# NVIDIA/retinanet-examples

Measured on AMD Instinct MI355X. Metric: images/sec end-to-end (incl. decode+NMS), RN50FPN 800px bs=8, higher is better.
Workload: dtype bf16; 1 GPU; ResNet50FPN bf16 inference, bs=8 per GPU at 800x1280, HIP decode x5 + NMS; global_batch=8, parallelism=replicas x1 (no data-path collective), entry=Model.forward (eval), postproc=fused

## Files before the change

include/odtk_hip.h:

```cpp
#ifndef ODTK_HIP_H
#define ODTK_HIP_H

#include <stddef.h>
#include <stdint.h>

#ifdef __cplusplus
extern "C" {
#endif

#define ODTK_OK                0
#define ODTK_ERR_INVALID      -1
#define ODTK_ERR_WORKSPACE    -2
#define ODTK_ERR_HIP          -3
#define ODTK_ERR_UNSUPPORTED  -4

#define ODTK_MAX_LEVELS    6
#define ODTK_MAX_ANCHORS   32
#define ODTK_ATSS_MAX_TOPK 16
#define ODTK_MAX_TOP_N     16384
#define ODTK_MAX_NMS_COUNT 7680
#define ODTK_MAX_NMS_COUNT_SCRATCH (1 << 22)
#define ODTK_MAX_NMS_DETECTIONS 2048

#define ODTK_F32   0
// ... 125 lines not shown
int odtk_preprocess_images(int batch_size, const odtk_image_t *images, const void *src, size_t src_bytes, const int32_t *tables,
                           size_t tables_len, const void *norm_table, void *out, int height, int width, int dtype, void *stream);

#define ODTK_AUGMENT_BRIGHTNESS 1u
#define ODTK_AUGMENT_CONTRAST   2u
#define ODTK_AUGMENT_HUE        4u
#define ODTK_AUGMENT_SATURATION 8u
typedef struct odtk_augment {
  int32_t canvas_width, canvas_height;
  int32_t map[6];
  uint32_t flags;
  float brightness, contrast, saturation;
  uint8_t hue;
  uint8_t pad_[3];
} odtk_augment_t;
int odtk_augment_images(int batch_size, const odtk_image_t *images, const odtk_augment_t *augments, const void *src, size_t src_bytes,
                        const int32_t *tables, size_t tables_len, const void *norm_table, void *out, int height, int width, int dtype,
                        void *workspace, size_t workspace_bytes, void *stream);
typedef struct odtk_rotation {
  double matrix[6];
  int32_t enabled;
  int32_t flip;
} odtk_rotation_t;
int odtk_augment_images_ex(int batch_size, const odtk_image_t *images, const odtk_augment_t *augments, const odtk_rotation_t *rotations,
                           const void *src, size_t src_bytes, const int32_t *tables, size_t tables_len, const void *norm_table, void *out,
                           int height, int width, int dtype, void *workspace, size_t workspace_bytes, void *stream);
int odtk_gemm_init(const char *hipblaslt_path);
size_t odtk_gemm_plan_export(char *text, size_t capacity);
int odtk_gemm_plan_import(const char *text);
int odtk_gemm_plan_pin_misses(void);
int odtk_gemm_bias_act(void *y, const void *x, const void *w, const float *bias, const void *residual,
                       size_t m, int n, int k, int dtype, int relu,
                       void *workspace, size_t workspace_size, void *stream);

int odtk_snap_to_anchors(int batch_size, const float *targets, int n_max, const float *anchors,
                         int num_anchors, int num_classes, int height, int width, int stride,
                         float iou_background, float iou_foreground,
                         float *cls_target, float *box_target, float *depth, void *stream);

typedef struct odtk_snap_level {
  const float *anchors;
  float *cls_target;
  float *box_target;
  float *depth;
  int32_t height, width, stride, pad_;
} odtk_snap_level_t;
int odtk_snap_to_anchors_levels(int batch_size, const float *targets, int n_max, int n_levels,
                                const odtk_snap_level_t *levels, int num_anchors, int num_classes,
                                float iou_background, float iou_foreground, void *stream);

int odtk_atss_assign_levels(int batch_size, const float *targets, int n_max, int n_levels,
                            const odtk_snap_level_t *levels, int num_anchors, int num_classes, int topk,
                            void *workspace, size_t workspace_size, void *stream);

typedef struct odtk_snap_rot_level {
  const float *anchors_axis;
  const float *anchors_quads;
  float *cls_target;
  float *box_target;
  float *depth;
  int32_t height, width, stride, pad_;
} odtk_snap_rot_level_t;
int odtk_snap_to_anchors_rotated_levels(int batch_size, const float *gt_axis, const float *gt_quads, const float *gt_class,
                                        int n_max, int n_levels, const odtk_snap_rot_level_t *levels, int num_anchors,
                                        int num_classes, float iou_background, float iou_foreground, void *stream);

// ... 15 lines not shown
  void *dcls, *dbox;
  int32_t height, width;
  int32_t channels_last;
  int32_t pad_;
} odtk_loss_level_t;

int odtk_retina_loss_levels_forward(int n_levels, const odtk_loss_level_t *levels, int batch_size, int num_anchors,
                                    int num_classes, int box_params, int dtype, float alpha, float gamma, float beta,
                                    double *sums, void *stream);
int odtk_retina_loss_levels_forward_ws(int n_levels, const odtk_loss_level_t *levels, int batch_size, int num_anchors,
                                       int num_classes, int box_params, int dtype, float alpha, float gamma, float beta,
                                       double *sums, void *workspace, size_t workspace_size, void *stream);
int odtk_retina_loss_levels_backward(int n_levels, const odtk_loss_level_t *levels, int batch_size, int num_anchors,
                                     int num_classes, int box_params, int dtype, float alpha, float gamma, float beta,
                                     const float *grad_cls_sums, const float *grad_box_sums, void *stream);

#define ODTK_KERNEL_PREFILTER 0
#define ODTK_KERNEL_SELECT    1
#define ODTK_KERNEL_NMS       2
#define ODTK_KERNEL_IOU       3
#define ODTK_KERNEL_EPILOGUE  4
#define ODTK_KERNEL_TARGETS   5
#define ODTK_KERNEL_GEMM      6
#define ODTK_KERNEL_LOSS      7
#define ODTK_KERNEL_SELHIST   8
#define ODTK_KERNEL_SELFILTER 9
#define ODTK_KERNEL_NMS_ORDER 10
#define ODTK_KERNEL_NMS_MATRIX 11
#define ODTK_KERNEL_POOL      12
#define ODTK_KERNEL_UPSAMPLE  13
#define ODTK_KERNEL_STEM_PACK 14
#define ODTK_KERNEL_LOSS_REDUCE 15
#define ODTK_KERNEL_ATSS_STATS 16
#define ODTK_KERNEL_COUNT     17
int odtk_profile_enable(int on);
int odtk_debug_set_trace(void *device_buffer);
int odtk_debug_loss_tuning(int which, int fp32_heads, int threads, int blocks_per_cu, int unroll, int box_blocks);
int odtk_debug_loss_layout(int which, int fp32_heads, int per_wave, int window, int box_rows);
int odtk_debug_loss_tuning_get(int which, int fp32_heads, int out[7]);
#define ODTK_LOSS_FORM_DEFAULT 1
int odtk_debug_loss_form(int form);
int odtk_debug_loss_form_get(void);
int odtk_profile_collect(double total_ms[ODTK_KERNEL_COUNT], int launches[ODTK_KERNEL_COUNT]);

#ifdef __cplusplus
}
#endif
#endif
```

retinanet-examples_amd/csrc/engine.hip:

```cpp
#include <cstring>

#include "runtime.hpp"
#include "epilogue.hpp"
#include "gemm_lt.hpp"

namespace {

template <typename T, bool kRes, bool kRelu>
int bias_act_launch(void *y, const float *bias, const void *res, uint64_t n, uint32_t channels, hipStream_t stream) {
  constexpr int per = T::kPerLoad;
  uint64_t done = 0;
  if (channels % per == 0 && n / per >= 256) {
    const uint32_t vpr = channels / per;
    const uint64_t n_vec = n / per;
    uint32_t g = vpr, m = 256;
    while (m) { const uint32_t r_ = g % m; g = m; m = r_; }
    const uint32_t unit = vpr / g;
    uint64_t blocks = (n_vec + 256ull * 4 - 1) / (256ull * 4);
    if (blocks > 256 * 16) blocks = 256 * 16;
    blocks = (blocks + unit - 1) / unit * unit;
    timed_launch(ODTK_KERNEL_EPILOGUE, odtk::bias_act_kernel<T, kRes, kRelu>, dim3(static_cast<unsigned>(blocks)), dim3(256), 0,
                 stream, y, bias, res, n_vec, vpr);
    done = n_vec * per;
  }
  if (done < n) {
    uint64_t blocks = (n - done + 255) / 256;
    if (blocks > 4096) blocks = 4096;
    hipLaunchKernelGGL((odtk::bias_act_scalar_kernel<T, kRes, kRelu>), dim3(static_cast<unsigned>(blocks)), dim3(256),
                       0, stream, y, bias, res, done, n, channels);
  }
  ODTK_HIP_TRY(hipGetLastError());
  return ODTK_OK;
}

template <typename T>
int bias_act_typed(void *y, const float *bias, const void *res, uint64_t n, uint32_t c, bool relu, hipStream_t s) {
  if (res) return relu ? bias_act_launch<T, true, true>(y, bias, res, n, c, s) : bias_act_launch<T, true, false>(y, bias, res, n, c, s);
  return relu ? bias_act_launch<T, false, true>(y, bias, res, n, c, s) : bias_act_launch<T, false, false>(y, bias, res, n, c, s);
}

int bias_act_dispatch(void *y, const float *bias, const void *res, uint64_t n, uint32_t c, int dtype, bool relu,
                      hipStream_t s) {
  return dispatch_dtype(dtype, [&](auto t) { return bias_act_typed<decltype(t)>(y, bias, res, n, c, relu, s); });
}

template <typename TIn>
int stem_pack_launch(const void *x, void *out, int batch, int height, int width, int channels_last, int out_dtype, hipStream_t stream) {
  const unsigned long long total = 1ull * batch * (height / 2) * (width / 2);
  unsigned long long blocks = (total + 255) / 256;
  if (blocks > 256 * 32) blocks = 256 * 32;
  const odtk::FastDiv by_wo = odtk::fastdiv_make(static_cast<uint32_t>(width / 2));
  const odtk::FastDiv by_howo = odtk::fastdiv_make(static_cast<uint32_t>(height / 2) * static_cast<uint32_t>(width / 2));
  if (out_dtype == ODTK_BF16)
    timed_launch(ODTK_KERNEL_STEM_PACK, odtk::stem_pack_kernel<TIn, odtk::BF16>, dim3(static_cast<unsigned>(blocks)), dim3(256), 0, stream, x, out,
                 static_cast<uint32_t>(batch), static_cast<uint32_t>(height), static_cast<uint32_t>(width), static_cast<uint32_t>(channels_last), by_wo, by_howo);
  else
    timed_launch(ODTK_KERNEL_STEM_PACK, odtk::stem_pack_kernel<TIn, odtk::F16>, dim3(static_cast<unsigned>(blocks)), dim3(256), 0, stream, x, out,
                 static_cast<uint32_t>(batch), static_cast<uint32_t>(height), static_cast<uint32_t>(width), static_cast<uint32_t>(channels_last), by_wo, by_howo);
  ODTK_HIP_TRY(hipGetLastError());
  return ODTK_OK;
}

}

extern "C" {

int odtk_bias_act(void *y, const float *bias, const void *residual, size_t n_pixels, int channels, int dtype,
                  int relu, void *stream) {
  if (!y || !bias || channels <= 0) return ODTK_ERR_INVALID;
  if (dtype != ODTK_F32 && dtype != ODTK_BF16 && dtype != ODTK_F16) return ODTK_ERR_UNSUPPORTED;
  if ((reinterpret_cast<uintptr_t>(y) & 15u) || (reinterpret_cast<uintptr_t>(residual) & 15u)) return ODTK_ERR_INVALID;
  const uint64_t n = static_cast<uint64_t>(n_pixels) * channels;
  if (n == 0) return ODTK_OK;
  return bias_act_dispatch(y, bias, residual, n, static_cast<uint32_t>(channels), dtype, relu != 0,
                           static_cast<hipStream_t>(stream));
}

int odtk_bias_act_maxpool(const void *y, const float *bias, void *out, int batch_size, int height, int width,
                          int channels, int dtype, int relu, void *stream) {
  if (!y || !bias || !out || batch_size <= 0 || height <= 0 || width <= 0 || channels <= 0) return ODTK_ERR_INVALID;
  if (dtype != ODTK_BF16 && dtype != ODTK_F16) return ODTK_ERR_UNSUPPORTED;
  if (channels % 8 != 0) return ODTK_ERR_UNSUPPORTED;
  if ((reinterpret_cast<uintptr_t>(y) | reinterpret_cast<uintptr_t>(out)) & 15u) return ODTK_ERR_INVALID;
  if (1ull * height * width * channels >= (1ull << 32)) return ODTK_ERR_UNSUPPORTED;
  const uint32_t ho = (static_cast<uint32_t>(height) + 1) / 2, wo = (static_cast<uint32_t>(width) + 1) / 2;
  const uint64_t work = static_cast<uint64_t>(batch_size) * ho * wo * (channels / 8);
  uint64_t blocks = (work + 255) / 256;
  if (blocks > 256 * 32) blocks = 256 * 32;
  hipStream_t s = static_cast<hipStream_t>(stream);
  const uint16_t *in = static_cast<const uint16_t *>(y);
  uint16_t *o = static_cast<uint16_t *>(out);
  odtk::PoolDivisors dv;
  dv.groups = odtk::fastdiv_make(static_cast<uint32_t>(channels / 8));
  dv.wo = odtk::fastdiv_make(wo);
  dv.ho = odtk::fastdiv_make(ho);
  const bool small = work < (1ull << 32);
#define ODTK_POOL_(T, R, S)                                                                                             \
  timed_launch(ODTK_KERNEL_POOL, odtk::bias_act_maxpool_kernel<T, R, S>, dim3(static_cast<unsigned>(blocks)), dim3(256), 0, s, in, \
// ... 103 lines not shown
```

retinanet-examples_amd/odtk/_C.py:

```python
import ctypes
import threading
import os

import torch

_LIB_PATH = os.environ.get('ODTK_HIP_LIBRARY') or os.path.join(os.path.dirname(os.path.abspath(__file__)), 'libodtk_hip.so')

OK, ERR_INVALID, ERR_WORKSPACE, ERR_HIP, ERR_UNSUPPORTED = 0, -1, -2, -3, -4
F32, BF16, F16 = 0, 1, 2
FLAG_ROTATED, FLAG_LOGITS, FLAG_ROTATED_NMS_FIXED_ANGLE = 1, 2, 4
MAX_LEVELS, MAX_ANCHORS, MAX_TOP_N, MAX_NMS_COUNT, MAX_NMS_COUNT_SCRATCH = 6, 32, 16384, 7680, 1 << 22
MAX_CONCAT_PARTS = 8
MAX_TILES = 64
SOFT_NMS_LINEAR, SOFT_NMS_GAUSSIAN = 1, 2
ATSS_MAX_TOPK = 16

_vp = ctypes.c_void_p
_vpp = ctypes.POINTER(ctypes.c_void_p)
_fp = ctypes.POINTER(ctypes.c_float)
_sz = ctypes.c_size_t


class LossLevel(ctypes.Structure):
    _fields_ = [('cls', ctypes.c_void_p), ('box', ctypes.c_void_p), ('depth', ctypes.c_void_p), ('box_target', ctypes.c_void_p),
# ... 92 lines not shown
    'odtk_snap_to_anchors_rotated_levels': (ctypes.c_int, [ctypes.c_int, _vp, _vp, _vp, ctypes.c_int, ctypes.c_int,
                                                           ctypes.POINTER(SnapRotLevel), ctypes.c_int, ctypes.c_int, ctypes.c_float,
                                                           ctypes.c_float, _vp]),
    'odtk_prefilter_thresholds': (ctypes.c_int, [_vp, ctypes.c_int, ctypes.c_int, ctypes.c_float, _vp, _vp]),
    'odtk_upsample_nearest2x': (ctypes.c_int, [ctypes.c_void_p, ctypes.c_void_p, ctypes.c_int, ctypes.c_int, ctypes.c_int, ctypes.c_int,
                                               ctypes.c_int, ctypes.c_void_p]),
    'odtk_canvas_clear': (ctypes.c_int, [ctypes.c_void_p] + [ctypes.c_int] * 5 + [ctypes.POINTER(ctypes.c_int), ctypes.c_int, ctypes.c_void_p]),
    'odtk_canvas_pack': (ctypes.c_int, [ctypes.c_void_p] + [ctypes.c_int] * 5 + [ctypes.POINTER(ctypes.c_int), _vpp, ctypes.c_int,
                                        ctypes.c_void_p]),
    'odtk_stem_pack': (ctypes.c_int, [ctypes.c_void_p, ctypes.c_void_p, ctypes.c_int, ctypes.c_int, ctypes.c_int, ctypes.c_int,
                                      ctypes.c_int, ctypes.c_int, ctypes.c_void_p]),
    'odtk_preprocess_images': (ctypes.c_int, [ctypes.c_int, ctypes.POINTER(Image), _vp, _sz, _vp, _sz, _vp, _vp, ctypes.c_int, ctypes.c_int,
                                              ctypes.c_int, _vp]),
    'odtk_augment_images': (ctypes.c_int, [ctypes.c_int, ctypes.POINTER(Image), ctypes.POINTER(Augment), _vp, _sz, _vp, _sz, _vp, _vp,
                                           ctypes.c_int, ctypes.c_int, ctypes.c_int, _vp, _sz, _vp]),
    'odtk_augment_images_ex': (ctypes.c_int, [ctypes.c_int, ctypes.POINTER(Image), ctypes.POINTER(Augment), ctypes.POINTER(Rotation), _vp, _sz,
                                              _vp, _sz, _vp, _vp, ctypes.c_int, ctypes.c_int, ctypes.c_int, _vp, _sz, _vp]),
    'odtk_nms_sorted_runs': (ctypes.c_int, [ctypes.c_int, _vpp, _vpp, ctypes.c_int, _sz, ctypes.c_int, _vp, ctypes.c_int, ctypes.c_float,
                                            ctypes.c_uint32, _vp, _sz, _vp]),
    'odtk_soft_nms': (ctypes.c_int, [ctypes.c_int, _vpp, _vpp, ctypes.c_int, _sz, ctypes.c_int, ctypes.c_float, ctypes.c_int,
                                     ctypes.c_float, ctypes.c_float, ctypes.c_uint32, _vp, _sz, _vp]),
    'odtk_box_vote': (ctypes.c_int, [ctypes.c_int, _vpp, _vp, _vp, _sz, ctypes.c_int, ctypes.c_float, ctypes.c_uint32, _vp]),
    'odtk_concat_candidates': (ctypes.c_int, [ctypes.c_int, ctypes.c_int, ctypes.POINTER(Candidates), _vpp, ctypes.c_uint32, _vp]),
    'odtk_tile_images': (ctypes.c_int, [_vp, _vp] + [ctypes.c_int] * 7 + [ctypes.POINTER(Tile), ctypes.c_int, ctypes.c_int, _vp]),
    'odtk_merge_tile_candidates': (ctypes.c_int, [ctypes.c_int, ctypes.POINTER(Tile), _vpp, _vpp, _sz] + [ctypes.c_int] * 6 +
                                   [ctypes.c_float, ctypes.c_uint32, _vp]),
    'odtk_gemm_init': (ctypes.c_int, [ctypes.c_char_p]),
    'odtk_gemm_plan_export': (ctypes.c_size_t, [ctypes.c_char_p, ctypes.c_size_t]),
    'odtk_gemm_plan_import': (ctypes.c_int, [ctypes.c_char_p]),
    'odtk_gemm_plan_pin_misses': (ctypes.c_int, []),
    'odtk_gemm_bias_act': (ctypes.c_int, [ctypes.c_void_p, ctypes.c_void_p, ctypes.c_void_p, ctypes.c_void_p, ctypes.c_void_p,
                                          ctypes.c_size_t, ctypes.c_int, ctypes.c_int, ctypes.c_int, ctypes.c_int,
                                          ctypes.c_void_p, ctypes.c_size_t, ctypes.c_void_p]),
    'odtk_profile_collect': (ctypes.c_int, [ctypes.POINTER(ctypes.c_double), ctypes.POINTER(ctypes.c_int)]),
}

KERNEL_NAMES = ('prefilter_scan_kernel', 'select_decode_kernel', 'nms_kernel', 'iou_pairs_kernel', 'bias_act_kernel',
                'snap_to_anchors_kernel', 'gemm_bias_act', 'retina_loss_kernel', 'select_hist_kernel', 'select_filter_kernel',
                'nms_first_round_kernel', 'rotated_sup_matrix_kernel', 'bias_act_maxpool_kernel', 'upsample_nearest2x_kernel',
                'stem_pack_kernel', 'loss_reduce_kernel', 'atss_stats_kernel')
traffic_count = False
traffic_bytes = {}


def _count(name, nbytes):
    if traffic_count:
        traffic_bytes[name] = traffic_bytes.get(name, 0) + int(nbytes)


_lib = None


def library():
    global _lib
    if _lib is None:
        if not os.path.isfile(_LIB_PATH):
            raise ImportError('odtk._C: %s is missing -- build the HIP library first '
                              '(python __graft_entry__.py, or make -C retinanet-examples_amd/csrc). '
                              'There is no CPU fallback.' % _LIB_PATH)
        lib = ctypes.CDLL(_LIB_PATH)
        for name, (res, args) in _SIGNATURES.items():
            fn = getattr(lib, name)
            fn.restype = res
            fn.argtypes = args
        for which, mirror in ((0, Level), (1, SnapLevel), (2, SnapRotLevel), (3, LossLevel), (5, Image), (6, Augment), (7, Rotation),
                              (9, Candidates), (11, Tile)):
            if lib.odtk_abi_struct_size(which) != ctypes.sizeof(mirror):
                raise ImportError('odtk._C: %s was built from another revision of include/odtk_hip.h (sizeof struct %d: library %d, '
                                  'binding %d) -- rebuild it (make -C retinanet-examples_amd/csrc)'
                                  % (_LIB_PATH, which, lib.odtk_abi_struct_size(which), ctypes.sizeof(mirror)))
        _lib = lib
        for part in filter(None, os.environ.get('ODTK_LOSS_TUNING', '').split(';')):
            side, _, vals = part.partition(':')
# ... 716 lines not shown
def gemm_available():
    if not _GEMM_READY:
        shipped = os.path.join(os.path.dirname(torch.__file__), 'lib', 'libhipblaslt.so')
        path = shipped if os.path.exists(shipped) else None
        rc = library().odtk_gemm_init(path.encode() if path else None)
        _GEMM_READY.append(rc == OK)
    return _GEMM_READY[0]


def gemm_bias_act(x, weight, bias, residual=None, relu=True):
    if not x.is_cuda or x.dim() != 4 or x.dtype not in _DTYPES:
        raise RuntimeError('gemm_bias_act: x must be a 4-d CUDA tensor of float32/bfloat16/float16')
    b, k, h, w = x.shape
    n = weight.shape[0]
    if weight.numel() != n * k or weight.dtype != x.dtype or not weight.is_contiguous() and not weight.is_contiguous(
            memory_format=torch.channels_last):
        raise RuntimeError('gemm_bias_act: weight must be a dense [Cout, Cin(, 1, 1)] tensor of x.dtype')
    if not _channels_last(x, True):
        raise RuntimeError('gemm_bias_act: x must be channels_last')
    if not _bias_vector(bias, n):
        raise RuntimeError('gemm_bias_act: bias must be a float32 CUDA vector of length Cout')
    y = torch.empty((b, n, h, w), dtype=x.dtype, device=x.device, memory_format=torch.channels_last)
    if residual is not None and (residual.shape != y.shape or residual.dtype != y.dtype or not _channels_last(residual, True)):
        raise RuntimeError('gemm_bias_act: residual must match the output (shape, dtype, channels_last)')
    with torch.cuda.device(x.device):
        ws, stream = _gemm_setup(x.device)
        _check(library().odtk_gemm_bias_act(y.data_ptr(), x.data_ptr(), weight.data_ptr(), bias.data_ptr(),
                                            residual.data_ptr() if residual is not None else None,
                                            b * h * w, n, k, _DTYPES[x.dtype], 1 if relu else 0,
                                            ws.data_ptr(), ws.numel(), stream), 'gemm_bias_act')
    return y


_CONV_LIB_PATH = os.path.join(os.path.dirname(os.path.abspath(__file__)), 'libodtk_conv.so')
_conv_lib = []


def conv_library():
    if not _conv_lib:
        lib = None
        if os.path.isfile(_CONV_LIB_PATH) and not os.environ.get('ODTK_NO_CONV_LIBRARY'):
            lib = ctypes.CDLL(_CONV_LIB_PATH)
            lib.odtk_conv_bias_act.restype = ctypes.c_int
            lib.odtk_conv_bias_act.argtypes = [ctypes.c_void_p] * 4 + [ctypes.c_int] * 13 + [ctypes.c_void_p]
            lib.odtk_conv_bias_act_pads.restype = ctypes.c_int
            lib.odtk_conv_bias_act_pads.argtypes = [ctypes.c_void_p] * 4 + [ctypes.c_int] * 15 + [ctypes.c_void_p]
            lib.odtk_conv_bias_act_strided.restype = ctypes.c_int
            lib.odtk_conv_bias_act_strided.argtypes = ([ctypes.c_void_p] * 4 + [ctypes.c_int] * 13 + [ctypes.c_longlong] * 6 +
                                                       [ctypes.c_int] * 2 + [ctypes.c_void_p])
            lib.odtk_conv_last_plan.restype = ctypes.c_char_p
            lib.odtk_conv_last_plan.argtypes = []
            lib.odtk_conv_instance_count.restype = ctypes.c_int
            lib.odtk_conv_instance_count.argtypes = [ctypes.c_int]
            lib.odtk_conv_plan_export.restype = ctypes.c_size_t
            lib.odtk_conv_plan_export.argtypes = [ctypes.c_char_p, ctypes.c_size_t]
            lib.odtk_conv_plan_import.restype = ctypes.c_int
            lib.odtk_conv_plan_import.argtypes = [ctypes.c_char_p]
        _conv_lib.append(lib)
    return _conv_lib[0]


def conv_available():
    return conv_library() is not None


def conv_bias_act(x, weight, bias, stride=(1, 1), padding=(1, 1), relu=True, out=None):
# ... 143 lines not shown
```

retinanet-examples_amd/odtk/fused.py:

```python
import hashlib
import json
import os
import threading

import torch
import torch.nn as nn
import torch.nn.functional as F

from . import _C
from . import box as box_ops
from .backbones.resnet import BasicBlock, Bottleneck


_PLAN_LOCK = threading.Lock()
_TLS = threading.local()


def _planning():
    return getattr(_TLS, 'planning', False)


def _key_str(key):
    kind, shape = ('only', key[1:]) if key and key[0] == 'only' else ('act', key)
    return kind + ':' + 'x'.join(str(int(v)) for v in shape)
# ... 183 lines not shown
    def _routed(self, key, kind, x, two, one):
        route = self.route.get(key)
        if route is None and _Conv.route_mode != 'auto':
            route = self.route[key] = (_Conv.route_mode == 'library', None, None)
        if route is None and _planning() and not torch.cuda.is_current_stream_capturing():
            route = self.route[key] = self._measure(x, two, one)
            self.learned[kind] = route[0]
        if route is None:
            return self.learned.get(kind, False)
        return route[0]

    def conv_then_pool(self, x):
        if not x.is_cuda:
            return F.max_pool2d(self._torch(x), 3, 2, 1)
        y = F.conv2d(x, self.weight, None, self.stride, self.padding, groups=self.groups)
        if y.dtype in (torch.bfloat16, torch.float16) and y.shape[1] % 8 == 0:
            return _C.bias_act_maxpool(y.contiguous(memory_format=torch.channels_last), self.bias, self.relu)
        return F.max_pool2d(_C.bias_act_(y.contiguous(memory_format=torch.channels_last), self.bias, None, self.relu), 3, 2, 1)


class _Block(nn.Module):
    def __init__(self, block, dtype):
        super().__init__()
        if isinstance(block, Bottleneck):
            self.convs = nn.ModuleList([_Conv(block.conv1, block.bn1, True, dtype), _Conv(block.conv2, block.bn2, True, dtype)])
            self.last = _Conv(block.conv3, block.bn3, True, dtype)
        elif isinstance(block, BasicBlock):
            self.convs = nn.ModuleList([_Conv(block.conv1, block.bn1, True, dtype)])
            self.last = _Conv(block.conv2, block.bn2, True, dtype)
        else:
            raise TypeError('unsupported block %r' % type(block))
        self.down = None if block.downsample is None else _Conv(block.downsample[0], block.downsample[1], False, dtype)

    def forward(self, x):
        skip = x if self.down is None else self.down(x)
        y = x
        for c in self.convs:
            y = c(y)
        return self.last(y, skip)


class FusedRetinaNet(nn.Module):
    @staticmethod
    def supports(model):
        if len(model.backbones) != 1:
            return False
        fpn = next(iter(model.backbones.values()))
        net = getattr(fpn, 'features', None)
        if net is None or not all(hasattr(net, n) for n in ('conv1', 'bn1', 'layer1', 'layer2', 'layer3', 'layer4')):
            return False
        if list(getattr(net, 'outputs', [])) != [3, 4, 5]:
            return False
        return all(isinstance(b, (Bottleneck, BasicBlock)) for layer in (net.layer1, net.layer2, net.layer3, net.layer4)
                   for b in layer)

    def __init__(self, model, dtype=torch.bfloat16):
        super().__init__()
        if not self.supports(model):
            raise ValueError('FusedRetinaNet supports a single ResNet-FPN backbone')
        fpn = next(iter(model.backbones.values()))
        net = fpn.features
        self.dtype = dtype
        self.model = [model]
        self.stem = _Conv(net.conv1, net.bn1, True, dtype)
        self.stem_s2d = None
        c1 = net.conv1
        if (tuple(c1.kernel_size), tuple(c1.stride), tuple(c1.padding), c1.in_channels, c1.groups) == ((7, 7), (2, 2), (3, 3), 3, 1) \
                and dtype in (torch.bfloat16, torch.float16):
            w = self.stem.weight.float()
            w4 = stem_space_to_depth_weights(w)
            self.register_buffer('stem_w4', w4.to(dtype).contiguous(memory_format=torch.channels_last))
            self.register_buffer('stem_zero_bias', torch.zeros(w.shape[0], dtype=dtype, device=w.device))
            self.stem_s2d = {}
        self.stem_learned = False
        self.layers = nn.ModuleList([nn.ModuleList([_Block(b, dtype) for b in layer])
                                     for layer in (net.layer1, net.layer2, net.layer3, net.layer4)])
        self.outputs = list(net.outputs)
        self.lateral = nn.ModuleList([_Conv(fpn.lateral3, None, False, dtype), _Conv(fpn.lateral4, None, False, dtype),
                                      _Conv(fpn.lateral5, None, False, dtype)])
        self.smooth = nn.ModuleList([_Conv(fpn.smooth3, None, False, dtype), _Conv(fpn.smooth4, None, False, dtype),
                                     _Conv(fpn.smooth5, None, False, dtype)])
        self.pyramid6 = _Conv(fpn.pyramid6, None, False, dtype)
        self.pyramid7 = _Conv(fpn.pyramid7, None, False, dtype)

        def head(seq):
            convs = [m for m in seq if isinstance(m, nn.Conv2d)]
            return nn.ModuleList([_Conv(c, None, i + 1 < len(convs), dtype) for i, c in enumerate(convs)])

        self.cls_head = head(model.cls_head)
        self.box_head = head(model.box_head)
        self.level_streams = True
        self.pyramid_canvas = os.environ.get('ODTK_PYRAMID_CANVAS', '1') != '0'
        self._streams = None
        self.tower_plan = 0
        self._planned = set()
        self._loaded_geometries = set()
        self._plan_file_seen = False
        self.libraries_taken = None
        self.max_plans = 4
        self._graphs = {}
        self._thresholds = {}
        self.max_graphs = 8

    def _stem_direct(self, x):
        x = x.to(self.dtype).contiguous(memory_format=torch.channels_last)
        return self.stem.conv_then_pool(x)

    def _stem_packed(self, x):
        xs = _C.stem_pack(x, self.dtype)
        y = _C.conv_bias_act(xs, self.stem_w4, self.stem_zero_bias, 1, ((2, 1), (2, 1)), False)
        return _C.bias_act_maxpool(y, self.stem.bias, self.stem.relu)

    def _stem(self, x):
        if (self.stem_s2d is not None and _Conv.use_conv_library and x.is_cuda and x.dim() == 4 and x.shape[1] == 3
                and x.shape[2] % 2 == 0 and x.shape[3] % 2 == 0 and x.dtype in _C._DTYPES and _C.conv_available()
                and (x.is_contiguous() or x.is_contiguous(memory_format=torch.channels_last))):
            key = (tuple(x.shape), x.dtype, x.is_contiguous())
            route = self.stem_s2d.get(key)
            if route is None and _Conv.route_mode != 'auto':
                route = self.stem_s2d[key] = (_Conv.route_mode == 'library', None, None)
            if route is None and _planning() and not torch.cuda.is_current_stream_capturing():
                route = self.stem_s2d[key] = self.stem._measure(x, self._stem_direct, self._stem_packed)
                self.stem_learned = route[0]
            if route[0] if route is not None else self.stem_learned:
                try:
                    return self._stem_packed(x)
                except RuntimeError:
                    self.stem_s2d[key] = (False, float('inf'), 0.0)
        return self._stem_direct(x)

    def features(self, x):
        x = self._stem(x)
        feats = []
        for level, layer in enumerate(self.layers, start=2):
            for block in layer:
                x = block(x)
            if level in self.outputs:
                feats.append(x)
        c3, c4, c5 = feats
        p5 = self.lateral[2](c5)
        p4 = self.lateral[1](c4, self._upsample(p5))
        p3 = self.lateral[0](c3, self._upsample(p4))
        p6 = self.pyramid6(c5)
        p7 = self.pyramid7(F.relu(p6))
        return [self.smooth[0](p3), self.smooth[1](p4), self.smooth[2](p5), p6, p7]

    @staticmethod
    def _upsample(t):
        if (t.is_cuda and t.dtype in _C._DTYPES and t.is_contiguous(memory_format=torch.channels_last)
                and (t.shape[1] * t.element_size()) % 16 == 0):
            return _C.upsample2x(t)
        return F.interpolate(t, scale_factor=2).contiguous(memory_format=torch.channels_last)

    @staticmethod
    def _run(seq, t):
        for c in seq:
            t = c(t)
        return t

    def _canvas_gutter(self, feats):
        if not self.pyramid_canvas or len(feats) < 3 or not (feats[0].is_cuda or self.pyramid_canvas == 'always'):
            return None
        gutter = 0
        for c in list(self.cls_head[:-1]) + list(self.box_head[:-1]):
            kh, kw = c.weight.shape[2:]
            if (tuple(c.stride) != (1, 1) or c.groups != 1 or kh % 2 == 0 or kw % 2 == 0 or tuple(c.padding) != (kh // 2, kw // 2)
                    or c.weight.shape[0] != c.weight.shape[1]):
                return None
            gutter = max(gutter, kh // 2, kw // 2)
# ... 67 lines not shown
        ready = torch.cuda.Event()
        ready.record(main)
        done = []
        for stream, group in zip(self._streams, groups):
            stream.wait_event(ready)
            with torch.cuda.stream(stream):
                for i in group:
                    for pair in unit(i):
                        for t in pair:
                            t.record_stream(main)
                e = torch.cuda.Event()
                e.record(stream)
                done.append(e)
        for i in mine:
            unit(i)
        for e in done:
            main.wait_event(e)
        return [o[0] for o in out], [o[1] for o in out]

    def heads(self, x):
        with torch.autocast(x.device.type, enabled=False):
            return self._towers(self.features(x), True)

    def heads_without_last_bias(self, x):
        with torch.autocast(x.device.type, enabled=False):
            cls, box = self._towers(self.features(x), False)
        return cls, box, self.cls_head[-1].bias, self.box_head[-1].bias

    @torch.no_grad()
    def replay(self, x):
        m = self.model[0]
        bias = self.cls_head[-1].bias
        key = (tuple(x.shape), x.dtype, x.device, x.is_contiguous(memory_format=torch.channels_last),
               m.threshold, m.top_n, m.nms, m.detections, self.level_streams, self.tower_plan, self.pyramid_canvas, bias.data_ptr(), bias._version,
               tuple(sorted(m.soft_nms.items())) if getattr(m, 'soft_nms', None) is not None else None,
               getattr(m, 'box_voting', None))
        if getattr(m, 'tta', None) is not None:
            raise RuntimeError('FusedRetinaNet.replay is not available with Model.tta (two passes of the engine)')
        if getattr(m, 'tile', None) is not None:
            raise RuntimeError('FusedRetinaNet.replay is not available with Model.tile (several passes of the engine)')
        entry = self._graphs.get(key)
        if entry is None:
            static_x = torch.empty_like(x)
            static_x.copy_(x)
            side = torch.cuda.Stream(x.device)
            side.wait_stream(torch.cuda.current_stream(x.device))
            with torch.cuda.stream(side):
                for _ in range(2):
                    self.forward(static_x)
            torch.cuda.current_stream(x.device).wait_stream(side)
            graph = torch.cuda.CUDAGraph()
            with torch.cuda.graph(graph):
                out = self.forward(static_x)
            while len(self._graphs) >= self.max_graphs:
                self._graphs.pop(next(iter(self._graphs)))
            entry = self._graphs[key] = (graph, static_x, out, tuple(self._thresholds.values()))
        graph, static_x, out = entry[:3]
        static_x.copy_(x)
        graph.replay()
        return tuple(o.clone() for o in out)

    def plan(self, x):
        path = os.environ.get('ODTK_CONV_PLAN')
        if path and not self._plan_file_seen:
            self._plan_file_seen = True
            if os.path.isfile(path):
                with open(path) as f:
# ... 121 lines not shown
```

Before: 1276 images/s.

## Fuse bottleneck last 1x1 conv with next block's first 1x1 conv in one kernel

Adds a HIP kernel that computes a ResNet bottleneck's final 1x1 conv (64->256, with bias, residual add and ReLU) and immediately feeds each output tile through the next block's first 1x1 conv (256->64/128) using MFMA with weights held in LDS. Both the block output and the next block's intermediate are written in one pass, so the 256-channel activation is not re-read from memory by a separate GEMM launch. Layer1/layer2 block boundaries with matching shapes use this path by default, falling back to the library convs on error. It trades the tuned hipBLASLt GEMMs for a hand-written persistent kernel whose efficiency is uncertain.

```diff
diff --git a/include/odtk_hip.h b/include/odtk_hip.h
--- a/include/odtk_hip.h
+++ b/include/odtk_hip.h
@@ -181,6 +181,8 @@
 int odtk_gemm_bias_act(void *y, const void *x, const void *w, const float *bias, const void *residual,
                        size_t m, int n, int k, int dtype, int relu,
                        void *workspace, size_t workspace_size, void *stream);
+int odtk_bottleneck_seam(void *out, void *z, const void *y2, const void *skip, const void *w3, const float *b3, const void *w1,
+                         const float *b1, size_t m, int c_in, int c_mid, int c_next, int dtype, void *stream);
 
 int odtk_snap_to_anchors(int batch_size, const float *targets, int n_max, const float *anchors,
                          int num_anchors, int num_classes, int height, int width, int stride,
@@ -262,7 +264,8 @@
 #define ODTK_KERNEL_STEM_PACK 14
 #define ODTK_KERNEL_LOSS_REDUCE 15
 #define ODTK_KERNEL_ATSS_STATS 16
-#define ODTK_KERNEL_COUNT     17
+#define ODTK_KERNEL_SEAM      17
+#define ODTK_KERNEL_COUNT     18
 int odtk_profile_enable(int on);
 int odtk_debug_set_trace(void *device_buffer);
 int odtk_debug_loss_tuning(int which, int fp32_heads, int threads, int blocks_per_cu, int unroll, int box_blocks);
diff --git a/retinanet-examples_amd/csrc/engine.hip b/retinanet-examples_amd/csrc/engine.hip
--- a/retinanet-examples_amd/csrc/engine.hip
+++ b/retinanet-examples_amd/csrc/engine.hip
@@ -3,6 +3,7 @@
 #include "runtime.hpp"
 #include "epilogue.hpp"
 #include "gemm_lt.hpp"
+#include "seam.hpp"
 
 namespace {
 
@@ -61,9 +62,49 @@
   return ODTK_OK;
 }
 
+template <typename T, int N2>
+int seam_launch(const void *y2, const void *skip, const void *w3, const float *b3, const void *w1, const float *b1, void *out, void *z,
+                uint64_t m, hipStream_t stream) {
+  constexpr size_t lds = odtk::seam_lds_bytes<N2>();
+  const int rc = allow_dynamic_lds(reinterpret_cast<const void *>(&odtk::bottleneck_seam_kernel<T, N2>), lds, "bottleneck_seam_kernel LDS");
+  if (rc != ODTK_OK) return rc;
+  int device = 0, cus = 0;
+  ODTK_HIP_TRY(hipGetDevice(&device));
+  ODTK_HIP_TRY(hipDeviceGetAttribute(&cus, hipDeviceAttributeMultiprocessorCount, device));
+  constexpr uint64_t per_group = odtk::kSeamThreads / 64 * 32;
+  uint64_t blocks = (m + per_group - 1) / per_group;
+  const uint64_t resident = static_cast<uint64_t>(cus > 0 ? cus : 1) * (160 * 1024 / lds);
+  if (blocks > resident) blocks = resident;
+  timed_launch(ODTK_KERNEL_SEAM, odtk::bottleneck_seam_kernel<T, N2>, dim3(static_cast<unsigned>(blocks)), dim3(odtk::kSeamThreads), lds, stream,
+               static_cast<const uint16_t *>(y2), static_cast<const uint16_t *>(skip), static_cast<const uint16_t *>(w3), b3,
+               static_cast<const uint16_t *>(w1), b1, static_cast<uint16_t *>(out), static_cast<uint16_t *>(z), m);
+  ODTK_HIP_TRY(hipGetLastError());
+  return ODTK_OK;
+}
+
 }
 
 extern "C" {
+
+int odtk_bottleneck_seam(void *out, void *z, const void *y2, const void *skip, const void *w3, const float *b3, const void *w1,
+                         const float *b1, size_t m, int c_in, int c_mid, int c_next, int dtype, void *stream) {
+  if (!out || !z || !y2 || !skip || !w3 || !b3 || !w1 || !b1 || c_in <= 0 || c_mid <= 0 || c_next <= 0) return ODTK_ERR_INVALID;
+  if (out == z || out == y2 || out == skip || z == y2 || z == skip) return ODTK_ERR_INVALID;
+  if (dtype != ODTK_BF16 && dtype != ODTK_F16) return ODTK_ERR_UNSUPPORTED;
+  if (c_in != odtk::kSeamCin || c_mid != odtk::kSeamCmid || (c_next != 64 && c_next != 128)) return ODTK_ERR_UNSUPPORTED;
+  if ((reinterpret_cast<uintptr_t>(out) | reinterpret_cast<uintptr_t>(z) | reinterpret_cast<uintptr_t>(y2) | reinterpret_cast<uintptr_t>(skip) |
+       reinterpret_cast<uintptr_t>(w3) | reinterpret_cast<uintptr_t>(w1)) & 15u)
+    return ODTK_ERR_INVALID;
+  if ((reinterpret_cast<uintptr_t>(b3) | reinterpret_cast<uintptr_t>(b1)) & 3u) return ODTK_ERR_INVALID;
+  if (m > (1ull << 40)) return ODTK_ERR_INVALID;
+  if (m == 0) return ODTK_OK;
+  hipStream_t s = static_cast<hipStream_t>(stream);
+  if (dtype == ODTK_BF16)
+    return c_next == 64 ? seam_launch<odtk::BF16, 64>(y2, skip, w3, b3, w1, b1, out, z, m, s)
+                        : seam_launch<odtk::BF16, 128>(y2, skip, w3, b3, w1, b1, out, z, m, s);
+  return c_next == 64 ? seam_launch<odtk::F16, 64>(y2, skip, w3, b3, w1, b1, out, z, m, s)
+                      : seam_launch<odtk::F16, 128>(y2, skip, w3, b3, w1, b1, out, z, m, s);
+}
 
 int odtk_bias_act(void *y, const float *bias, const void *residual, size_t n_pixels, int channels, int dtype,
                   int relu, void *stream) {
diff --git a/retinanet-examples_amd/csrc/seam.hpp b/retinanet-examples_amd/csrc/seam.hpp
--- /dev/null
+++ b/retinanet-examples_amd/csrc/seam.hpp
@@ -0,0 +1,218 @@
+#pragma once
+
+#include "common.hpp"
+#include "prefilter.hpp"
+
+namespace odtk {
+
+typedef float seam_f32x16 __attribute__((ext_vector_type(16)));
+typedef __bf16 seam_bf16x8 __attribute__((ext_vector_type(8)));
+typedef _Float16 seam_f16x8 __attribute__((ext_vector_type(8)));
+typedef __bf16 seam_bf16x2 __attribute__((ext_vector_type(2)));
+typedef _Float16 seam_f16x2 __attribute__((ext_vector_type(2)));
+typedef float seam_f32x2 __attribute__((ext_vector_type(2)));
+typedef float seam_f32x4 __attribute__((ext_vector_type(4)));
+
+constexpr int kSeamThreads = 256;
+constexpr int kSeamCin = 64, kSeamCmid = 256;
+
+template <int N2>
+constexpr size_t seam_lds_bytes() {
+  return 8 * 4 * 64 * 16 + 8 * 2 * (N2 / 32) * 64 * 16 + (kSeamCmid + N2) * 4 + (kSeamThreads / 64) * 256 * 16;
+}
+
+__device__ __forceinline__ uint32_t seam_pi(uint32_t rho) {
+  return (rho & ~12u) | ((rho & 4u) << 1) | ((rho & 8u) >> 1);
+}
+
+template <typename T>
+__device__ __forceinline__ seam_f32x16 seam_mfma(vuint4 a, vuint4 b, seam_f32x16 c) {
+  if constexpr (std::is_same_v<T, BF16>)
+    return __builtin_amdgcn_mfma_f32_32x32x16_bf16(__builtin_bit_cast(seam_bf16x8, a), __builtin_bit_cast(seam_bf16x8, b), c, 0, 0, 0);
+  else
+    return __builtin_amdgcn_mfma_f32_32x32x16_f16(__builtin_bit_cast(seam_f16x8, a), __builtin_bit_cast(seam_f16x8, b), c, 0, 0, 0);
+}
+
+template <typename T>
+__device__ __forceinline__ uint32_t seam_pack2(float lo, float hi) {
+  if constexpr (std::is_same_v<T, BF16>)
+    return __builtin_bit_cast(uint32_t, __builtin_convertvector(seam_f32x2{lo, hi}, seam_bf16x2));
+  else
+    return __builtin_bit_cast(uint32_t, __builtin_convertvector(seam_f32x2{lo, hi}, seam_f16x2));
+}
+
+template <typename T>
+__device__ __forceinline__ float seam_unpack(uint32_t word, int half) {
+  const uint32_t h = half ? word >> 16 : word & 0xffffu;
+  return std::is_same_v<T, BF16> ? bf16_bits_to_float(h) : f16_bits_to_float(h);
+}
+
+template <typename T, bool kSkip>
+__device__ __forceinline__ vuint4 seam_epilogue(const seam_f32x16 &acc, int u, const float *bias8, vuint4 skip) {
+  const seam_f32x4 b0 = *reinterpret_cast<const seam_f32x4 *>(bias8), b1 = *reinterpret_cast<const seam_f32x4 *>(bias8 + 4);
+  float v[8];
+#pragma unroll
+  for (int e = 0; e < 8; ++e) {
+    float o = acc[8 * u + e];
+    if (kSkip) o += seam_unpack<T>(skip[e >> 1], e & 1);
+    o += e < 4 ? b0[e & 3] : b1[e & 3];
+    v[e] = o > 0.0f ? o : (o != o ? o : 0.0f);
+  }
+  vuint4 r;
+#pragma unroll
+  for (int d = 0; d < 4; ++d) r[d] = seam_pack2<T>(v[2 * d], v[2 * d + 1]);
+  return r;
+}
+
+struct SeamPanel {
+  vuint4 *stage;
+  uint32_t row[4];
+  uint32_t pix[4];
+  uint32_t chunk;
+  uint32_t frag_base, frag_swz;
+  __device__ __forceinline__ SeamPanel(vuint4 *stage_, uint32_t lane) : stage(stage_) {
+#pragma unroll
+    for (uint32_t i = 0; i < 4; ++i) {
+      const uint32_t e = 64 * i + lane;
+      pix[i] = e >> 3;
+      row[i] = (e & ~7u) | ((e & 7u) ^ ((e >> 4) & 7u));
+    }
+    chunk = lane & 7u;
+    const uint32_t r = lane & 31u;
+    frag_base = 8 * r;
+    frag_swz = (r >> 1) & 7u;
+  }
+  __device__ __forceinline__ uint32_t frag(uint32_t c) const { return frag_base + (c ^ frag_swz); }
+};
+
+template <bool kStream>
+__device__ __forceinline__ void seam_load_panel(vuint4 (&v)[4], const SeamPanel &pn, const uint16_t *base, uint32_t row_elems, uint32_t col,
+                                                uint64_t tile, uint64_t m) {
+#pragma unroll
+  for (int i = 0; i < 4; ++i) {
+    uint64_t p = tile * 32 + pn.pix[i];
+    p = p < m ? p : m - 1;
+    const vuint4 *src = reinterpret_cast<const vuint4 *>(base + p * row_elems + col) + pn.chunk;
+    v[i] = kStream ? __builtin_nontemporal_load(src) : *src;
+  }
+}
+
+template <bool kFull>
+__device__ __forceinline__ void seam_store_panel(const SeamPanel &pn, uint16_t *base, uint32_t row_elems, uint32_t col, uint64_t tile,
+                                                 uint64_t m) {
+#pragma unroll
+  for (int i = 0; i < 4; ++i) {
+    const uint64_t p = tile * 32 + pn.pix[i];
+    const vuint4 v = pn.stage[pn.row[i]];
+    if (kFull || p < m) *(reinterpret_cast<vuint4 *>(base + p * row_elems + col) + pn.chunk) = v;
+  }
+}
+
+template <typename T, int N2, bool kFull>
+__device__ __forceinline__ void seam_tile(const SeamPanel &pn, uint32_t lane, const vuint4 *s_w3, const vuint4 *s_w1, const float *s_b3,
+                                          const float *s_b1, vuint4 (&yq)[4], vuint4 (&sq)[4][4], const uint16_t *y2, const uint16_t *skip,
+                                          uint16_t *out, uint16_t *z, uint64_t tile, uint64_t next, uint64_t m) {
+  constexpr int NT = N2 / 32;
+  const uint32_t h = lane >> 5;
+  vuint4 yf[4];
+#pragma unroll
+  for (int i = 0; i < 4; ++i) pn.stage[pn.row[i]] = yq[i];
+#pragma unroll
+  for (int s = 0; s < 4; ++s) yf[s] = pn.stage[pn.frag(2 * s + h)];
+  seam_load_panel<false>(yq, pn, y2, kSeamCin, 0, next, m);
+
+  seam_f32x16 zacc[NT];
+#pragma unroll
+  for (int t = 0; t < NT; ++t)
+#pragma unroll
+    for (int e = 0; e < 16; ++e) zacc[t][e] = 0.0f;
+
+#pragma unroll
+  for (int q = 0; q < 4; ++q) {
+    asm volatile("" ::: "memory");
+#pragma unroll
+    for (int i = 0; i < 4; ++i) pn.stage[pn.row[i]] = sq[q][i];
+    seam_load_panel<true>(sq[q], pn, skip, kSeamCmid, 64 * q, next, m);
+#pragma unroll
+    for (int b = 0; b < 2; ++b) {
+      const int blk = 2 * q + b;
+      seam_f32x16 x;
+#pragma unroll
+      for (int e = 0; e < 16; ++e) x[e] = 0.0f;
+#pragma unroll
+      for (int s = 0; s < 4; ++s) x = seam_mfma<T>(s_w3[(blk * 4 + s) * 64 + lane], yf[s], x);
+#pragma unroll
+      for (int u = 0; u < 2; ++u) {
+        const uint32_t at = pn.frag(4 * b + 2 * u + h);
+        const vuint4 frag = seam_epilogue<T, true>(x, u, s_b3 + 32 * blk + 16 * u + 8 * h, pn.stage[at]);
+        pn.stage[at] = frag;
+#pragma unroll
+        for (int t = 0; t < NT; ++t) zacc[t] = seam_mfma<T>(s_w1[((blk * 2 + u) * NT + t) * 64 + lane], frag, zacc[t]);
+      }
+    }
+    seam_store_panel<kFull>(pn, out, kSeamCmid, 64 * q, tile, m);
+  }
+#pragma unroll
+  for (int g = 0; g < NT / 2; ++g) {
+    asm volatile("" ::: "memory");
+#pragma unroll
+    for (int b = 0; b < 2; ++b) {
+#pragma unroll
+      for (int u = 0; u < 2; ++u)
+        pn.stage[pn.frag(4 * b + 2 * u + h)] =
+            seam_epilogue<T, false>(zacc[2 * g + b], u, s_b1 + 32 * (2 * g + b) + 16 * u + 8 * h, vuint4{0u, 0u, 0u, 0u});
+    }
+    seam_store_panel<kFull>(pn, z, N2, 64 * g, tile, m);
+  }
+}
+
+template <typename T, int N2>
+__global__ __launch_bounds__(kSeamThreads) void bottleneck_seam_kernel(const uint16_t *__restrict__ y2, const uint16_t *__restrict__ skip,
+                                                                       const uint16_t *__restrict__ w3, const float *__restrict__ b3,
+                                                                       const uint16_t *__restrict__ w1, const float *__restrict__ b1,
+                                                                       uint16_t *__restrict__ out, uint16_t *__restrict__ z, uint64_t m) {
+  constexpr int NT = N2 / 32;
+  extern __shared__ __attribute__((aligned(16))) unsigned char seam_lds[];
+  vuint4 *s_w3 = reinterpret_cast<vuint4 *>(seam_lds);
+  vuint4 *s_w1 = s_w3 + 8 * 4 * 64;
+  float *s_b3 = reinterpret_cast<float *>(s_w1 + 8 * 2 * NT * 64);
+  float *s_b1 = s_b3 + kSeamCmid;
+  vuint4 *s_stage = reinterpret_cast<vuint4 *>(s_b1 + N2);
+
+  const uint32_t tid = threadIdx.x, lane = tid & 63u;
+  for (uint32_t f = tid; f < 8 * 4 * 64; f += kSeamThreads) {
+    const uint32_t fl = f & 63u, s = (f >> 6) & 3u, blk = f >> 8;
+    const uint32_t row = 32 * blk + seam_pi(fl & 31u), k = 16 * s + 8 * (fl >> 5);
+    s_w3[f] = *reinterpret_cast<const vuint4 *>(w3 + row * kSeamCin + k);
+  }
+  for (uint32_t f = tid; f < 8 * 2 * NT * 64; f += kSeamThreads) {
+    const uint32_t fl = f & 63u, t = (f >> 6) % NT, bs = (f >> 6) / NT;
+    const uint32_t row = 32 * t + seam_pi(fl & 31u), k = 16 * bs + 8 * (fl >> 5);
+    s_w1[f] = *reinterpret_cast<const vuint4 *>(w1 + row * kSeamCmid + k);
+  }
+  for (uint32_t c = tid; c < kSeamCmid + N2; c += kSeamThreads) s_b3[c] = c < kSeamCmid ? b3[c] : b1[c - kSeamCmid];
+  __syncthreads();
+
+  const uint64_t n_tiles = (m + 31) / 32, n_full = m / 32;
+  const uint64_t stride = static_cast<uint64_t>(gridDim.x) * (kSeamThreads / 64);
+  uint64_t tile = static_cast<uint64_t>(blockIdx.x) * (kSeamThreads / 64) + (tid >> 6);
+  if (tile >= n_tiles) return;
+
+  const SeamPanel pn(s_stage + (tid >> 6) * 256, lane);
+  vuint4 yq[4], sq[4][4];
+  seam_load_panel<false>(yq, pn, y2, kSeamCin, 0, tile, m);
+#pragma unroll
+  for (int q = 0; q < 4; ++q) {
+    asm volatile("" ::: "memory");
+    seam_load_panel<true>(sq[q], pn, skip, kSeamCmid, 64 * q, tile, m);
+  }
+  asm volatile("" ::: "memory");
+#pragma unroll 1
+  for (; tile < n_full; tile += stride) {
+    const uint64_t next = tile + stride < n_tiles ? tile + stride : tile;
+    seam_tile<T, N2, true>(pn, lane, s_w3, s_w1, s_b3, s_b1, yq, sq, y2, skip, out, z, tile, next, m);
+  }
+  if (tile < n_tiles) seam_tile<T, N2, false>(pn, lane, s_w3, s_w1, s_b3, s_b1, yq, sq, y2, skip, out, z, tile, tile, m);
+}
+
+}
diff --git a/retinanet-examples_amd/odtk/_C.py b/retinanet-examples_amd/odtk/_C.py
--- a/retinanet-examples_amd/odtk/_C.py
+++ b/retinanet-examples_amd/odtk/_C.py
@@ -148,13 +148,14 @@
     'odtk_gemm_bias_act': (ctypes.c_int, [ctypes.c_void_p, ctypes.c_void_p, ctypes.c_void_p, ctypes.c_void_p, ctypes.c_void_p,
                                           ctypes.c_size_t, ctypes.c_int, ctypes.c_int, ctypes.c_int, ctypes.c_int,
                                           ctypes.c_void_p, ctypes.c_size_t, ctypes.c_void_p]),
+    'odtk_bottleneck_seam': (ctypes.c_int, [ctypes.c_void_p] * 8 + [ctypes.c_size_t] + [ctypes.c_int] * 4 + [ctypes.c_void_p]),
     'odtk_profile_collect': (ctypes.c_int, [ctypes.POINTER(ctypes.c_double), ctypes.POINTER(ctypes.c_int)]),
 }
 
 KERNEL_NAMES = ('prefilter_scan_kernel', 'select_decode_kernel', 'nms_kernel', 'iou_pairs_kernel', 'bias_act_kernel',
                 'snap_to_anchors_kernel', 'gemm_bias_act', 'retina_loss_kernel', 'select_hist_kernel', 'select_filter_kernel',
                 'nms_first_round_kernel', 'rotated_sup_matrix_kernel', 'bias_act_maxpool_kernel', 'upsample_nearest2x_kernel',
-                'stem_pack_kernel', 'loss_reduce_kernel', 'atss_stats_kernel')
+                'stem_pack_kernel', 'loss_reduce_kernel', 'atss_stats_kernel', 'bottleneck_seam_kernel')
 traffic_count = False
 traffic_bytes = {}
 
@@ -937,6 +938,28 @@
     return y
 
 
+def bottleneck_seam(y2, skip, w3, b3, w1, b1):
+    if not y2.is_cuda or y2.dim() != 4 or y2.dtype not in (torch.bfloat16, torch.float16):
+        raise RuntimeError('bottleneck_seam: y2 must be a 4-d CUDA tensor of bfloat16/float16')
+    b, k, h, w = y2.shape
+    c, n = w3.shape[0], w1.shape[0]
+    for name, wt, rows, cols in (('w3', w3, c, k), ('w1', w1, n, c)):
+        if wt.numel() != rows * cols or wt.shape[1] != cols or wt.dtype != y2.dtype or wt.device != y2.device or not (
+                wt.is_contiguous() or wt.is_contiguous(memory_format=torch.channels_last)):
+            raise RuntimeError('bottleneck_seam: %s must be a dense [%d, %d(, 1, 1)] tensor of y2.dtype' % (name, rows, cols))
+    if skip.shape != (b, c, h, w) or skip.dtype != y2.dtype or skip.device != y2.device or not _channels_last(skip, True) \
+            or not _channels_last(y2, True):
+        raise RuntimeError('bottleneck_seam: y2 and skip must be channels_last, skip [B, %d, H, W] of y2.dtype' % c)
+    if not _bias_vector(b3, c) or not _bias_vector(b1, n):
+        raise RuntimeError('bottleneck_seam: b3 / b1 must be float32 CUDA vectors of length %d / %d' % (c, n))
+    out = torch.empty((b, c, h, w), dtype=y2.dtype, device=y2.device, memory_format=torch.channels_last)
+    z = torch.empty((b, n, h, w), dtype=y2.dtype, device=y2.device, memory_format=torch.channels_last)
+    _launch(library().odtk_bottleneck_seam, 'bottleneck_seam', y2.device, out.data_ptr(), z.data_ptr(), y2.data_ptr(), skip.data_ptr(),
+            w3.data_ptr(), b3.data_ptr(), w1.data_ptr(), b1.data_ptr(), b * h * w, k, c, n, _DTYPES[y2.dtype])
+    _count('bottleneck_seam_kernel', (y2.numel() + skip.numel() + out.numel() + z.numel()) * y2.element_size())
+    return out, z
+
+
 _CONV_LIB_PATH = os.path.join(os.path.dirname(os.path.abspath(__file__)), 'libodtk_conv.so')
 _conv_lib = []
 
diff --git a/retinanet-examples_amd/odtk/fused.py b/retinanet-examples_amd/odtk/fused.py
--- a/retinanet-examples_amd/odtk/fused.py
+++ b/retinanet-examples_amd/odtk/fused.py
@@ -239,12 +239,24 @@
             raise TypeError('unsupported block %r' % type(block))
         self.down = None if block.downsample is None else _Conv(block.downsample[0], block.downsample[1], False, dtype)
 
-    def forward(self, x):
+    def forward(self, x, z=None, seam=None):
         skip = x if self.down is None else self.down(x)
-        y = x
-        for c in self.convs:
+        y = x if z is None else z
+        for c in (self.convs if z is None else self.convs[1:]):
             y = c(y)
-        return self.last(y, skip)
+        if seam is None:
+            return self.last(y, skip)
+        try:
+            return _C.bottleneck_seam(y, skip, self.last.weight, self.last.bias, seam.weight, seam.bias)
+        except RuntimeError:
+            out = self.last(y, skip)
+            return out, seam(out)
+
+    def seam_to(self, nxt, dtype):
+        last, first = self.last, nxt.convs[0]
+        return (len(self.convs) == 2 and dtype in (torch.bfloat16, torch.float16)
+                and all(c.pointwise and tuple(c.stride) == (1, 1) and c.relu for c in (last, first))
+                and tuple(last.weight.shape[:2]) == (256, 64) and tuple(first.weight.shape[:2]) in ((64, 256), (128, 256)))
 
 
 class FusedRetinaNet(nn.Module):
@@ -282,6 +294,9 @@
         self.stem_learned = False
         self.layers = nn.ModuleList([nn.ModuleList([_Block(b, dtype) for b in layer])
                                      for layer in (net.layer1, net.layer2, net.layer3, net.layer4)])
+        blocks = [b for layer in self.layers for b in layer]
+        self._seams = {a: b for a, b in zip(blocks, blocks[1:]) if a.seam_to(b, dtype)}
+        self.seam_fusion = os.environ.get('ODTK_SEAM_FUSION', '1') != '0'
         self.outputs = list(net.outputs)
         self.lateral = nn.ModuleList([_Conv(fpn.lateral3, None, False, dtype), _Conv(fpn.lateral4, None, False, dtype),
                                       _Conv(fpn.lateral5, None, False, dtype)])
@@ -339,9 +354,11 @@
     def features(self, x):
         x = self._stem(x)
         feats = []
+        z = None
         for level, layer in enumerate(self.layers, start=2):
             for block in layer:
-                x = block(x)
+                nxt = self._seams.get(block) if self.seam_fusion and x.is_cuda else None
+                x, z = block(x, z, nxt.convs[0]) if nxt is not None else (block(x, z), None)
             if level in self.outputs:
                 feats.append(x)
         c3, c4, c5 = feats
@@ -475,7 +492,7 @@
         m = self.model[0]
         bias = self.cls_head[-1].bias
         key = (tuple(x.shape), x.dtype, x.device, x.is_contiguous(memory_format=torch.channels_last),
-               m.threshold, m.top_n, m.nms, m.detections, self.level_streams, self.tower_plan, self.pyramid_canvas, bias.data_ptr(), bias._version,
+               m.threshold, m.top_n, m.nms, m.detections, self.level_streams, self.tower_plan, self.pyramid_canvas, self.seam_fusion, bias.data_ptr(), bias._version,
                tuple(sorted(m.soft_nms.items())) if getattr(m, 'soft_nms', None) is not None else None,
                getattr(m, 'box_voting', None))
         if getattr(m, 'tta', None) is not None:
```

New measurement: 1314 images/s, median of 6. 3.0% higher.
